# zgchen33/MCGaze

Hardware: AMD Instinct MI355X
Metric: clips/sec (7x3x224x224) (higher is better)
Workload: dtype f16x3; 1 GPU; full multiclue_gaze_r50 forward (R-50 + FPN + 4 decoder stages + gaze head), 64 clips/GPU x 7 frames x 3x224x224, 64 clips/step; clips_per_gpu=64, clip_length=7, global_clips=64, chunk_frames=0, parallelism=single GPU, trunk_streams=2

## Files before the change

include/mcgaze_hip.h:

```cpp
#ifndef MCGAZE_HIP_H
#define MCGAZE_HIP_H

#include <stddef.h>
#include <stdint.h>

#ifdef __cplusplus
extern "C" {
#endif

#define MCG_ABI_VERSION 19

enum { MCG_OK = 0, MCG_ERR_ARG = 1, MCG_ERR_HIP = 2, MCG_ERR_UNSUPPORTED = 3, MCG_ERR_WORKSPACE = 4 };
typedef enum { MCG_F32 = 0, MCG_BF16 = 1, MCG_F16X3 = 2, MCG_F16 = 3 } mcg_dtype;
#define MCG_ELEM_BYTES(dt) (((dt) == MCG_BF16 || (dt) == MCG_F16) ? 2 : 4)
typedef void* mcg_stream;

int mcg_abi_version(void);
const char* mcg_build_id(void);
const char* mcg_last_error(void);
int mcg_device_info(int* cu_count, size_t* hbm_bytes, char* arch, int arch_len);

int mcg_nchw_to_nhwc(mcg_stream s, mcg_dtype dt, const float* src, void* dst, int N, int C, int H, int W);
int mcg_nhwc_to_nchw(mcg_stream s, mcg_dtype dt, const void* src, float* dst, int N, int C, int H, int W);

// ... 11 lines not shown
  void* y;
  int N, H, W, Cin, Cout, KH, KW, stride, pad;
  int relu;
  int residual_mode;
  int Hr, Wr;
  const void* x2;
  int Cin2, stride2, H2, W2;
  int tile;
  int flags;
  float wscale;
} mcg_conv_desc;
int mcg_conv2d(mcg_stream s, mcg_dtype dt, const mcg_conv_desc* d);

int mcg_bottleneck_x3(mcg_stream s, const float* x, const float* src2, const void* wstream, const float* bias, float* y, float* z,
                      int frames, int H, int W, int cm, int nsrc, int cn, void* trace);

size_t mcg_conv3x3_wino_x3_weight_bytes(int Cin, int Cout, int g);
int mcg_conv3x3_wino_x3(mcg_stream s, const float* x, const void* u, const float* bias, float* y, int frames, int H, int W,
                        int Cin, int Cout, int relu, int tile, float wscale, int g);

int mcg_pointwise_stream(mcg_stream s, mcg_dtype dt, const void* a, const void* wf, const float* bias, const void* res, void* y,
                         int M, int K, int N, int relu, int res_mode, int Ho, int Wo, int Hr, int Wr, float wscale,
                         const int* block_list, const int* block_count, int grid_cap);
int mcg_pointwise_dyn(mcg_stream s, mcg_dtype dt, const void* a, const void* wf, const float* bias, void* y, int M, float wscale, int grid_cap);
int mcg_pointwise_pair(mcg_stream s, mcg_dtype dt, const void* a1, const void* a2, const void* res, const void* w3f, const float* b3,
                       void* y, const void* w1f, const float* b1, void* z, int M, int K2, int C2, int grid_cap);

size_t mcg_stem_workspace_bytes(mcg_dtype dt, int N, int H, int W);
int mcg_stem_forward(mcg_stream s, mcg_dtype dt, const float* img, const void* w_stem, const float* bias,
                     void* y, int N, int H, int W, void* ws, size_t ws_bytes, int flags);
// ... 268 lines not shown
```

mcgaze_amd/csrc/bneck_x3.hpp:

```cpp
#pragma once
#include "igemm_dma.hpp"

#ifndef BNX_ABLATE
#define BNX_ABLATE 0
#endif
namespace bnx {
constexpr int TH = 8, TW = 28, WH = TH + 2, WW = TW + 2;
constexpr int NPIX = TH * TW, NG = NPIX / 32, WPIX = WH * WW;
constexpr int PLANE = WPIX * 16 + 32;
constexpr int NPLANE = 16;
constexpr int WIN_BYTES = NPLANE * PLANE;
constexpr int SLAB = 16384, NSLOT = 5, RING_BYTES = NSLOT * SLAB;
constexpr int NCOMP = NG, NT = 64 * (NCOMP + 1);
constexpr int WIN_ROUNDS = (WPIX * 16 + NCOMP * 64 - 1) / (NCOMP * 64);
static_assert(NPIX % 32 == 0, "tile must be whole 32-pixel groups");
}

struct BneckParams {
  const float* x;
  const float* res;
  const char* wstream;
  const float* bias;
  float* y;
  float* z;
  int H, W, tiles_x, tiles_per_frame, total_tiles;
  int res_blocked, y_blocked;
  unsigned long long* trace;
};

__device__ __forceinline__ void bnx_split8(const float (&v)[8], bf16x8& hi, bf16x8& lo) {
  uint32_t h[4], l[4];
#pragma unroll
  for (int q = 0; q < 4; ++q) split_pair(v[2 * q], v[2 * q + 1], h[q], l[q]);
  hi = __builtin_bit_cast(bf16x8, make_uint4(h[0], h[1], h[2], h[3]));
  lo = __builtin_bit_cast(bf16x8, make_uint4(l[0], l[1], l[2], l[3]));
}

__device__ __forceinline__ void bnx_step(const char* sl, const bf16x8& xh, const bf16x8& xl, f32x16& a0, f32x16& a1) {
  const bf16x8 w0h = __builtin_bit_cast(bf16x8, *(const uint4*)(sl));
  const bf16x8 w0l = __builtin_bit_cast(bf16x8, *(const uint4*)(sl + 1024));
  const bf16x8 w1h = __builtin_bit_cast(bf16x8, *(const uint4*)(sl + 8192));
  const bf16x8 w1l = __builtin_bit_cast(bf16x8, *(const uint4*)(sl + 8192 + 1024));
// ... 1 lines not shown
  a1 = x3_mfma(w1l, xh, a1);
  a0 = x3_mfma(w0h, xl, a0);
  a1 = x3_mfma(w1h, xl, a1);
  a0 = x3_mfma(w0h, xh, a0);
  a1 = x3_mfma(w1h, xh, a1);
}

__device__ __forceinline__ void bnx_barrier_drained() {
  asm volatile("s_waitcnt lgkmcnt(0)" ::: "memory");
  __builtin_amdgcn_s_barrier();
}

template <int CM, int NSRC, int CN, int LAYOUT>
__global__ __launch_bounds__(bnx::NT, 1) void bneck_x3_kernel(const BneckParams p) {
  using namespace bnx;
  constexpr bool RES_BLK = (LAYOUT & 1) != 0, Y_BLK = (LAYOUT & 2) != 0;
  static_assert(!RES_BLK || NSRC == 1, "only a residual can arrive blocked");
  constexpr int C = 4 * CM, KH = CM / 64, NCH = C / 64;
  constexpr int PARTS = CM / 64 + NSRC - 1;
  constexpr int NS1 = 9 * KH * KH;
  constexpr int NS = NS1 + NCH * (PARTS + CN / 64);
  constexpr int CT1 = CM / 32, CT3 = CN / 32;
  constexpr int WPC = (WIN_ROUNDS + NCH - 1) / NCH;
  constexpr int RD = 1;
  static_assert(NCH % RD == 0, "chunk loop is unrolled by the prefetch depth");
  static_assert(CM == 64 || CM == 128, "64 or 128 mid channels");
  static_assert(NSRC == 1 || CM == 64, "the second source is layer1's first block only");
  extern __shared__ __attribute__((aligned(16))) char smem[];
  char* const s_win = smem;
  char* const s_ring = smem + WIN_BYTES;
  float* const s_bias = (float*)(smem + WIN_BYTES + RING_BYTES);
  const int tid = threadIdx.x, lane = tid & 63;
  const int wave = __builtin_amdgcn_readfirstlane(tid >> 6);
  for (int i = tid; i < CM + C + CN + 4; i += NT) s_bias[i] = p.bias[i];
  __syncthreads();
  const int first = blockIdx.x, stride = gridDim.x;
  if (first >= p.total_tiles) return;

  if (wave == NCOMP) {
    const u32x4 srd_w = make_srd(p.wstream);
    const uint32_t ring_base = (uint32_t)(uintptr_t)(__attribute__((address_space(3))) char*)s_ring;
    const uint32_t voff = (uint32_t)lane * 16u;
    uint32_t kt_issue = 0, slot_issue = 0;
    int issued_total = 0;
    auto issue = [&]() {
      const uint32_t src = kt_issue * SLAB, dst = ring_base + slot_issue * SLAB;
      if (!(BNX_ABLATE & 1) || issued_total < NSLOT || p.H < 0)
        static_for<16>([&](auto pc) { lds_dma16<decltype(pc)::value * 1024>(voff, srd_w, src + decltype(pc)::value * 1024, dst); });
      if (BNX_ABLATE & 1) ++issued_total;
// ... 53 lines not shown
    ty0 = tyi * TH;
    tx0 = (r - tyi * p.tiles_x) * TW;
  };
  auto win_load = [&](int t, int kh, int it) -> float4 {
    int n, ty0, tx0;
    origin(t, n, ty0, tx0);
    const int idx = it * (NCOMP * 64) + ctid;
    const int wp = idx >> 4, c16 = idx & 15;
    const int wy = wp / WW, wx = wp - wy * WW;
    const int gy = ty0 - 1 + wy, gx = tx0 - 1 + wx;
    float4 v = make_float4(0.f, 0.f, 0.f, 0.f);
    if (idx < WPIX * 16 && (unsigned)gy < (unsigned)p.H && (unsigned)gx < (unsigned)p.W)
      v = *(const float4*)(p.x + (((long long)n * p.H + gy) * p.W + gx) * CM + kh * 64 + c16 * 4);
    return v;
  };
  auto win_park = [&](int it, const float4& v) {
    const int idx = it * (NCOMP * 64) + ctid;
    if (idx >= WPIX * 16) return;
    const int wp = idx >> 4, c16 = idx & 15;
    uint32_t h0, l0, h1, l1;
    split_pair(v.x, v.y, h0, l0);
    split_pair(v.z, v.w, h1, l1);
    char* dst = s_win + (((c16 >> 2) * 2 + ((c16 >> 1) & 1)) * 2) * PLANE + wp * 16 + (c16 & 1) * 8;
    *(uint2*)dst = make_uint2(h0, h1);
    *(uint2*)(dst + PLANE) = make_uint2(l0, l1);
  };

  for (int it = 0; it < WIN_ROUNDS; ++it) win_park(it, win_load(first, 0, it));

  const uint32_t a_lane = (uint32_t)lane * 16u;
  uint32_t slot = 0;
  auto slab_at = [&](int i) { const uint32_t t = slot + i; return s_ring + (t >= NSLOT ? t - NSLOT : t) * SLAB + a_lane; };
  auto slab_adv = [&](int n) { slot = slot + n >= NSLOT ? slot + n - NSLOT : slot + n; };

  int tr_c = 0;
  auto stamp = [&]() {
    if (p.trace && blockIdx.x == 0 && tid == 0 && tr_c < 2040) { p.trace[tr_c] = __builtin_amdgcn_s_memtime(); ++tr_c; }
  };
  for (int tile = first; tile < p.total_tiles; tile += stride) {
    stamp();
    int n, ty0, tx0;
    origin(tile, n, ty0, tx0);
    const int gy = ty0 + ty, gx = tx0 + tx;
    const bool valid = gy < p.H && gx < p.W;
    const bool st_ok = valid && ((BNX_ABLATE & 4) ? p.H < 0 : true), ld_ok = valid && ((BNX_ABLATE & 2) ? p.H < 0 : true);
    const long long row = ((long long)n * p.H + (valid ? gy : 0)) * p.W + (valid ? gx : 0);
    const long long sblk = ((long long)tile * NG + g) * (32 * C);
    const uint32_t lane_off = (uint32_t)(pl * 8 + 4 * half);
    const int next = tile + stride;
    const bool has_next = next < p.total_tiles && ((BNX_ABLATE & 8) ? p.H < 0 : true);

    float4 rres[RD][2][4];
    bf16x8 xfh[4], xfl[4];
    auto res_load = [&](auto slotc, int chunk) {
      constexpr int SL = decltype(slotc)::value;
#pragma unroll
      for (int c = 0; c < 2; ++c)
#pragma unroll
        for (int q = 0; q < 4; ++q)
          rres[SL][c][q] = !ld_ok ? make_float4(0.f, 0.f, 0.f, 0.f)
                                  : (RES_BLK ? *(const float4*)(p.res + sblk + lane_off + chunk * 2048 + c * 1024 + q * 256)
                                                   : *(const float4*)(p.res + row * C + chunk * 64 + c * 32 + 8 * q + 4 * half));
    };
// ... 2 lines not shown
    } else {
#pragma unroll
      for (int s = 0; s < 4; ++s) {
        const float4 a = valid ? *(const float4*)(p.res + row * 64 + 16 * s + 4 * half) : make_float4(0.f, 0.f, 0.f, 0.f);
        const float4 b = valid ? *(const float4*)(p.res + row * 64 + 16 * s + 4 * half + 8) : make_float4(0.f, 0.f, 0.f, 0.f);
        const float v[8] = {a.x, a.y, a.z, a.w, b.x, b.y, b.z, b.w};
        bnx_split8(v, xfh[s], xfl[s]);
      }
    }

    float4 w2nd[KH == 2 ? WIN_ROUNDS : 1];
    const bool win2 = (BNX_ABLATE & 8) ? (p.H < 0 || tile == first) : true;
    if constexpr (KH == 2) {
      if (win2) {
#pragma unroll
        for (int it = 0; it < WIN_ROUNDS; ++it) w2nd[it] = win_load(tile, 1, it);
      }
    }
    f32x16 acc1[CT1];
#pragma unroll
    for (int c = 0; c < CT1; ++c)
#pragma unroll
      for (int r = 0; r < 16; ++r) acc1[c][r] = 0.f;
    asm volatile("s_waitcnt lgkmcnt(0)" ::: "memory");
    static_for<KH>([&](auto khc) {
      constexpr int KHI = decltype(khc)::value;
      if constexpr (KHI == 1) {
        bnx_barrier_drained();
        if (win2) {
#pragma unroll
          for (int it = 0; it < WIN_ROUNDS; ++it) win_park(it, w2nd[it]);
        }
        asm volatile("s_waitcnt lgkmcnt(0)" ::: "memory");
      }
      static_for<9>([&](auto tc) {
        constexpr int TAP = decltype(tc)::value;
        constexpr int TOFF = ((TAP / 3) * WW + TAP % 3) * 16;
        bnx_barrier_drained();
        const char* sl[CM / 64];
#pragma unroll
        for (int op = 0; op < CM / 64; ++op) sl[op] = slab_at(op);
        static_for<4>([&](auto jc) {
          constexpr int J = decltype(jc)::value;
          const bf16x8 xh = __builtin_bit_cast(bf16x8, *(const uint4*)(bw + (4 * J) * PLANE + TOFF));
          const bf16x8 xl = __builtin_bit_cast(bf16x8, *(const uint4*)(bw + (4 * J + 1) * PLANE + TOFF));
          static_for<CM / 64>([&](auto opc) {
            constexpr int OP = decltype(opc)::value;
            bnx_step(sl[OP] + J * 2048, xh, xl, acc1[2 * OP], acc1[2 * OP + 1]);
          });
        });
        slab_adv(CM / 64);
      });
    });
    stamp();
    bf16x8 tfh[CM / 16], tfl[CM / 16];
#pragma unroll
    for (int s = 0; s < CM / 16; ++s) {
      const int c = s >> 1, q0 = 2 * (s & 1);
      float v[8];
#pragma unroll
// ... 9 lines not shown

    f32x16 acc3[CT3 > 0 ? CT3 : 1];
#pragma unroll
    for (int c = 0; c < (CT3 > 0 ? CT3 : 1); ++c)
#pragma unroll
      for (int r = 0; r < 16; ++r) acc3[c][r] = 0.f;
#pragma unroll 1
    for (int oc0 = 0; oc0 < NCH; oc0 += RD)
    static_for<RD>([&](auto occ) {
      constexpr int SLOT = decltype(occ)::value;
      const int oc = oc0 + SLOT;
      float4 wv[WPC];
      if (has_next) {
#pragma unroll
        for (int j = 0; j < WPC; ++j)
          if (oc * WPC + j < WIN_ROUNDS) wv[j] = win_load(next, 0, oc * WPC + j);
      }
      f32x16 acc2[2];
#pragma unroll
      for (int c = 0; c < 2; ++c)
#pragma unroll
        for (int r = 0; r < 16; ++r) acc2[c][r] = 0.f;
      bnx_barrier_drained();
      static_for<PARTS>([&](auto pc) {
        constexpr int PART = decltype(pc)::value;
        const char* sl = slab_at(PART);
        static_for<4>([&](auto sc) {
          constexpr int S = decltype(sc)::value;
          const bf16x8 bh = PART < CM / 64 ? tfh[(PART < CM / 64 ? PART : 0) * 4 + S] : xfh[S];
          const bf16x8 bl = PART < CM / 64 ? tfl[(PART < CM / 64 ? PART : 0) * 4 + S] : xfl[S];
          bnx_step(sl + S * 2048, bh, bl, acc2[0], acc2[1]);
// ... 70 lines not shown
static inline int launch_bneck_x3_t(hipStream_t s, const BneckParams& p) {
  constexpr int kLds = bnx::WIN_BYTES + bnx::RING_BYTES + (CM + 4 * CM + CN + 4) * 4;
  int cus;
  if (kernel_ready<bneck_x3_kernel<CM, NSRC, CN, LAYOUT>>(kLds, &cus)) return 1;
  const int grid = p.total_tiles < cus ? p.total_tiles : cus;
  hipLaunchKernelGGL((bneck_x3_kernel<CM, NSRC, CN, LAYOUT>), dim3(grid), dim3(bnx::NT), kLds, s, p);
  return hipGetLastError() == hipSuccess ? 0 : 1;
}
static inline bool bneck_x3_layout_ok(int cm, int nsrc, int cn, int res_blocked, int y_blocked) {
  return (!res_blocked || nsrc == 1) && (!y_blocked || (cn == cm));
}
static inline int launch_bneck_x3(hipStream_t s, BneckParams p, int frames, int cm, int nsrc, int cn) {
  const int tiles_y = (p.H + bnx::TH - 1) / bnx::TH;
  p.tiles_x = (p.W + bnx::TW - 1) / bnx::TW;
  p.tiles_per_frame = tiles_y * p.tiles_x;
  const long long total = (long long)p.tiles_per_frame * frames;
  if (total <= 0 || total > 0x7fffffffLL) return 1;
  p.total_tiles = (int)total;
  if (!bneck_x3_layout_ok(cm, nsrc, cn, p.res_blocked, p.y_blocked)) return 1;
  const int lay = (p.res_blocked ? 1 : 0) | (p.y_blocked ? 2 : 0);
  if (cm == 128) {
    if (cn == 0) return lay ? launch_bneck_x3_t<128, 1, 0, 1>(s, p) : launch_bneck_x3_t<128, 1, 0, 0>(s, p);
    switch (lay) {
      case 0: return launch_bneck_x3_t<128, 1, 128, 0>(s, p);
      case 1: return launch_bneck_x3_t<128, 1, 128, 1>(s, p);
      case 2: return launch_bneck_x3_t<128, 1, 128, 2>(s, p);
      default: return launch_bneck_x3_t<128, 1, 128, 3>(s, p);
    }
  }
  if (nsrc == 1) {
    if (cn == 0) return lay ? launch_bneck_x3_t<64, 1, 0, 1>(s, p) : launch_bneck_x3_t<64, 1, 0, 0>(s, p);
    if (cn == 128) return lay ? launch_bneck_x3_t<64, 1, 128, 1>(s, p) : launch_bneck_x3_t<64, 1, 128, 0>(s, p);
    switch (lay) {
      case 0: return launch_bneck_x3_t<64, 1, 64, 0>(s, p);
      case 1: return launch_bneck_x3_t<64, 1, 64, 1>(s, p);
      case 2: return launch_bneck_x3_t<64, 1, 64, 2>(s, p);
      default: return launch_bneck_x3_t<64, 1, 64, 3>(s, p);
    }
  }
  if (cn == 0) return launch_bneck_x3_t<64, 2, 0, 0>(s, p);
  if (cn == 64) return lay ? launch_bneck_x3_t<64, 2, 64, 2>(s, p) : launch_bneck_x3_t<64, 2, 64, 0>(s, p);
  return launch_bneck_x3_t<64, 2, 128, 0>(s, p);
// ... 2 lines not shown
```

mcgaze_amd/csrc/engine.hip:

```cpp
#include "igemm.hpp"
#include "pw_pair.hpp"
#include "pw_single.hpp"
#include "bneck_x3.hpp"
#include "pw_single_x3.hpp"
#include "wino_x3.hpp"

#include <stdarg.h>
#include <stdlib.h>
#include <string.h>

#include <map>
#include <mutex>
#include <string>
#include <vector>

int launch_roi_align(hipStream_t s, mcg_dtype dt, const void* const feats[4], const int feat_h[4], const int feat_w[4],
                     const int strides[4], int C, const float* boxes, int num_boxes, int boxes_per_frame, const int32_t* frame_of,
                     int pyramid_frames, void* out, int32_t* levels_out);
int launch_init_queries(hipStream_t s, mcg_dtype dt, const float* init_boxes, const void* init_feats, const int* img_hw,
                        const int32_t* frame_of, int pyramid_frames, int H, int W, float* boxes, void* obj, int N);
bool roi_mark_supported(int H, int W);
int launch_defer_clear(hipStream_t s, int* p, int n);
int launch_roi_mark(hipStream_t s, const float* boxes, int num_boxes, int boxes_per_frame, int level, int H, int W, int stride, int* state,
                    int* list, int* count);
int launch_inner_mark(hipStream_t s, const int* out_list, const int* out_count, int H, int W, int nblk, int* state, int* list, int* count);

struct mcg_engine {
  mcg_dtype dt;
  int blocks[4];
  mcg_conv_weights stem;
  std::vector<mcg_conv_weights> convs;
  mcg_conv_weights lateral[4], fpn_out[4], c3_ds[4];
  std::vector<mcg_fused_block> fused;
  bool bneck_fused = true;
  bool bneck_blocked = true;
  int winograd = 1;
  int wino_tile = -1;
  int fpn_deferred = 1;
  int fpn_lateral_deferred = 1;
  static constexpr int kAuditCap = 256;
  unsigned long long* audit_dev = nullptr;
  std::vector<std::string> audit_names;
  const float* init_boxes;
  const void* init_feats;
  int num_stages;
  std::vector<const void*> stage_w;
  const void* gaze_w[MCG_GW_COUNT];
  float stds[4];
  static constexpr int kMaxSplit = 4, kCandidates = 8;
  struct StreamPool* pool = nullptr;
// ... 120 lines not shown
extern "C" int mcg_engine_set_option(mcg_engine* e, const char* name, int value) {
  MCG_CHECK_ARG(e && name, "mcg_engine_set_option: null pointer");
  std::lock_guard<std::mutex> lock(e->mu);
  if (!strcmp(name, "trunk_streams")) { MCG_CHECK_ARG(value >= 1 && value <= mcg_engine::kMaxSplit, "trunk_streams must be 1..%d", mcg_engine::kMaxSplit); e->trunk_streams = value; }
  else if (!strcmp(name, "max_range_frames")) { MCG_CHECK_ARG(value >= 0, "max_range_frames must be >= 0"); e->max_range_frames = value; }
  else if (!strcmp(name, "tile")) e->ctx.tile = value > 0 ? value : -1;
  else if (!strcmp(name, "staged_gemm")) e->ctx.staged = value != 0;
  else if (!strcmp(name, "conv3x3_c64")) e->ctx.c64 = value != 0;
  else if (!strcmp(name, "stem_fused")) e->ctx.stem_fused = value != 0;
  else if (!strcmp(name, "decoder_chain")) e->ctx.chain = value != 0;
  else if (!strcmp(name, "decoder_attn_block")) e->ctx.attn_block = value != 0;
  else if (!strcmp(name, "pointwise_pair")) e->pw_pair = value != 0;
  else if (!strcmp(name, "pointwise_stream")) e->pw_single = value != 0;
  else if (!strcmp(name, "bottleneck_fused")) e->bneck_fused = value != 0;
  else if (!strcmp(name, "bottleneck_blocked")) e->bneck_blocked = value != 0;
  else if (!strcmp(name, "winograd")) { MCG_CHECK_ARG(value >= 0 && value <= 2, "winograd must be 0, 1 or 2"); e->winograd = value; }
  else if (!strcmp(name, "fpn_deferred")) e->fpn_deferred = value != 0;
  else if (!strcmp(name, "fpn_lateral_deferred")) e->fpn_lateral_deferred = value != 0;
  else if (!strcmp(name, "wino_tile")) { MCG_CHECK_ARG(value >= -1 && value <= 3, "wino_tile must be -1 (by grid size) .. 3"); e->wino_tile = value; }
  else if (!strcmp(name, "range_audit")) {
    MCG_CHECK_ARG(!mcg_is16(e->dt) || !value, "range_audit: f32-storage engines only (MCG_F32, MCG_F16X3)");
    if (value && !e->audit_dev) {
      if (hipMalloc((void**)&e->audit_dev, sizeof(unsigned long long) * 2 * mcg_engine::kAuditCap) != hipSuccess) { e->audit_dev = nullptr; mcg_set_error("range_audit: hipMalloc failed"); return MCG_ERR_HIP; }
    }
    if (value && hipMemset(e->audit_dev, 0, sizeof(unsigned long long) * 2 * mcg_engine::kAuditCap) != hipSuccess) { mcg_set_error("range_audit: hipMemset failed"); return MCG_ERR_HIP; }
    if (!value && e->audit_dev) { (void)hipFree(e->audit_dev); e->audit_dev = nullptr; }
    e->audit_names.clear();
  }
  else { mcg_set_error("mcg_engine_set_option: unknown option '%s'", name); return MCG_ERR_ARG; }
  return MCG_OK;
// ... 195 lines not shown
  const bool ds = b == 0;
  const mcg_conv_weights &d2 = e->convs[ci + 1], &d3 = e->convs[ci + 2];
  const int kk = ds ? e->convs[ci + 3].cin : 0, ss = ds ? e->convs[ci + 3].stride : 1;
  const int cn_i = ci + (ds ? 4 : 3);
  const bool nx = f->cn == 0 || (cn_i < (int)e->convs.size() && e->convs[cn_i].k == 1 && e->convs[cn_i].stride == 1 && e->convs[cn_i].cout == f->cn && e->convs[cn_i].cin == f->c);
  return (d2.k == 3 && d2.stride == 1 && d2.pad == 1 && d2.cin == f->cm && d2.cout == f->cm && d3.cout == f->c && f->nsrc == (ds ? 2 : 1) && nx &&
          bneck_x3_applicable(f->cm, f->c, f->cn, f->nsrc, kk, ss)) ? f : nullptr;
}
static int fused_tail_step(const mcg_engine* e, hipStream_t s, const TrunkWs& t, AuditCursor& au, TrunkCursor& c, const mcg_fused_block* fb,
                           int n, int l, int b, void* y) {
  const bool has_ds = b == 0;
  const int k2 = has_ds ? e->convs[c.ci + 3].cin : 0;
  BneckParams bp;
  memset(&bp, 0, sizeof(bp));
  bp.x = (const float*)c.o1; bp.res = (const float*)c.x; bp.wstream = (const char*)fb->wstream; bp.bias = fb->bias;
  bp.y = (float*)y; bp.z = (float*)c.o2; bp.H = c.h; bp.W = c.w;
  const long long blk_bytes = (long long)n * ((c.h + bnx::TH - 1) / bnx::TH) * ((c.w + bnx::TW - 1) / bnx::TW) * bnx::NPIX * fb->c * (long long)esize(e->dt);
  const mcg_fused_block* fnext = (b + 1 < e->blocks[l]) ? fused_tail_at(e, c.ci + (has_ds ? 4 : 3), b + 1) : nullptr;
  bp.res_blocked = c.x_blocked ? 1 : 0;
  bp.y_blocked = (e->bneck_blocked && !e->audit_dev && y != (void*)t.c[l] && fb->cn > 0 && fnext && fnext->nsrc == 1 && fnext->c == fb->c &&
                  blk_bytes <= (long long)t.big) ? 1 : 0;
  const double M = (double)n * c.h * c.w;
  ProfRec* rec = prof_begin(e->ctx, s, 70, n * c.h * c.w, fb->c + fb->cn, 9 * fb->cm + fb->cm + k2 + fb->c,
                            2.0 * M * (9.0 * fb->cm * fb->cm + (double)(fb->cm + k2) * fb->c + (double)fb->c * fb->cn),
                            4.0 * (M * (fb->cm + (has_ds ? k2 : fb->c) + fb->c + fb->cn) + 9.0 * fb->cm * fb->cm + (double)(fb->cm + k2) * fb->c + (double)fb->c * fb->cn));
  MCG_TRY(launch_done(rec, s, launch_bneck_x3(s, bp, n, fb->cm, fb->nsrc, fb->cn), "bneck_x3"));
  audit_tensor(au, y, (long long)n * c.h * c.w * fb->c, "layer%d.%d.out (fused tail)", l + 1, b);
  if (fb->cn > 0) {
    audit_tensor(au, c.o2, (long long)n * c.h * c.w * fb->cn, "layer%d.%d.next_conv1 (fused tail)", l + 1, b);
    std::swap(c.o1, c.o2);
    c.o1_ready = true;
// ... 252 lines not shown
      if (hipStreamWaitEvent(si[i], e->ev_fork, 0) != hipSuccess) { mcg_set_error("mcg_backbone_fpn_forward: hipStreamWaitEvent failed"); return MCG_ERR_HIP; }
  }
  const size_t part_ws = k > 1 ? al256(trunk_layout(e->dt, per, H, W, nullptr).total) : 0;
  int rc = MCG_OK;
  for (int f0 = 0, i = 0; f0 < N && rc == MCG_OK; f0 += per, i = (i + 1) % k)
    rc = trunk_chunk(e, si[i], img, f0, (N - f0) < per ? (N - f0) : per, H, W, pyramid, (char*)ws + (size_t)i * part_ws, backbone_only, tk);
  for (int i = 1; i < k; ++i) {
    if (hipEventRecord(e->ev_join[i - 1], si[i]) != hipSuccess || hipStreamWaitEvent(s, e->ev_join[i - 1], 0) != hipSuccess) {
      mcg_set_error("mcg_backbone_fpn_forward: join failed");
      rc = rc == MCG_OK ? MCG_ERR_HIP : rc;
    }
  }
  return rc;
}

extern "C" int mcg_bottleneck_x3(mcg_stream s, const float* x, const float* src2, const void* wstream, const float* bias, float* y, float* z,
                                 int frames, int H, int W, int cm, int nsrc, int cn, void* trace) {
  MCG_CHECK_ARG(x && src2 && wstream && bias && y && (z || cn == 0), "mcg_bottleneck_x3: null pointer");
  MCG_CHECK_ARG(frames > 0 && H > 0 && W > 0, "mcg_bottleneck_x3: empty problem");
  MCG_CHECK_ARG(bneck_x3_applicable(cm, 4 * cm, cn, nsrc, 64, 1), "mcg_bottleneck_x3: unsupported shape (cm=%d nsrc=%d cn=%d)", cm, nsrc, cn);
  BneckParams bp;
  memset(&bp, 0, sizeof(bp));
  bp.x = x; bp.res = src2; bp.wstream = (const char*)wstream; bp.bias = bias; bp.y = y; bp.z = z; bp.H = H; bp.W = W; bp.trace = (unsigned long long*)trace;
  if (launch_bneck_x3((hipStream_t)s, bp, frames, cm, nsrc, cn)) { mcg_set_error("mcg_bottleneck_x3: launch failed"); return MCG_ERR_HIP; }
  return MCG_OK;
}

extern "C" size_t mcg_conv3x3_wino_x3_weight_bytes(int Cin, int Cout, int g) {
  return (Cin > 0 && Cout > 0 && Cin % 32 == 0 && Cout % wnx::UNT == 0 && (g == 2 || g == 4)) ? wino_x3_weight_bytes(Cin, Cout, g) : 0;
}
extern "C" int mcg_conv3x3_wino_x3(mcg_stream s, const float* x, const void* u, const float* bias, float* y, int frames, int H, int W,
                                   int Cin, int Cout, int relu, int tile, float wscale, int g) {
  MCG_CHECK_ARG(x && u && y, "mcg_conv3x3_wino_x3: null pointer");
  MCG_CHECK_ARG(tile >= 0 && tile <= 4, "mcg_conv3x3_wino_x3: tile must be 0 (by grid size) .. 4");
  if (!wino_x3_applicable(frames, H, W, Cin, Cout, g)) {
    mcg_set_error("mcg_conv3x3_wino_x3: unsupported shape (frames=%d %dx%d, %d -> %d channels, F(%d,3)): Cin %% 32, Cout %% 128, W <= 62 (F(4,3): W %% 4 == 0, W >= 16), a tile's window within its buffer", frames, H, W, Cin, Cout, g);
    return MCG_ERR_UNSUPPORTED;
  }
  WinoParams wp;
  memset(&wp, 0, sizeof(wp));
// ... 236 lines not shown
```

mcgaze_amd/engine.py:

```python
import ctypes as C
import os

import numpy as np
import torch

from . import lib as L
from .packing import PackedWeights

_TORCH_DT = {'bf16': torch.bfloat16, 'f16': torch.float16, 'fp16': torch.float16, 'fp32': torch.float32, 'f32': torch.float32, 'f16x3': torch.float32, 'bf16x3': torch.float32}
_CODE = {'bf16': L.MCG_BF16, 'f16': L.MCG_F16, 'fp16': L.MCG_F16, 'fp32': L.MCG_F32, 'f32': L.MCG_F32, 'f16x3': L.MCG_F16X3,
         'bf16x3': L.MCG_F16X3}


def _code(dtype):
    return L.MCG_BF16 if dtype == torch.bfloat16 else (L.MCG_F16 if dtype == torch.float16 else L.MCG_F32)


def _ptr(t):
    return C.c_void_p(t.data_ptr()) if t is not None else C.c_void_p(0)


def _stream(device=None):
    return C.c_void_p(torch.cuda.current_stream(device).cuda_stream)

# ... 107 lines not shown

def conv3x3_wino(x, w, bias=None, relu=False, tile=0, g=2):
    _require_gpu()
    lib = L.load()
    from .packing import pow2_prescale, wino_pack
    N, H, W, Cin = x.shape
    Cout = w.shape[0]
    ws, wscale = pow2_prescale(w.cpu())
    u = wino_pack(ws, g=g).to(x.device)
    assert u.numel() * 2 == lib.mcg_conv3x3_wino_x3_weight_bytes(Cin, Cout, g), (u.numel(), Cin, Cout)
    y = torch.empty(N, H, W, Cout, dtype=torch.float32, device=x.device)
    L.check(lib.mcg_conv3x3_wino_x3(_stream(), _ptr(x.contiguous()), _ptr(u), _ptr(bias), _ptr(y), N, H, W, Cin, Cout, int(relu), tile, wscale, g), 'mcg_conv3x3_wino_x3')
    return y


def bottleneck_x3(x, src2, wstream, bias, cn, nsrc, trace=None):
    _require_gpu()
    lib = L.load()
    N, H, W, cm = x.shape
    y = torch.empty(N, H, W, 4 * cm, dtype=torch.float32, device=x.device)
    z = torch.empty(N, H, W, cn, dtype=torch.float32, device=x.device) if cn else None
    L.check(lib.mcg_bottleneck_x3(_stream(), _ptr(x.contiguous()), _ptr(src2.contiguous()), _ptr(wstream), _ptr(bias), _ptr(y), _ptr(z),
                                  N, H, W, cm, nsrc, cn, _ptr(trace)), 'mcg_bottleneck_x3')
    return y, z


def stem(img, w_stem, bias, dtype, flags=0, split=False):
    _require_gpu()
    lib = L.load()
    N, _, H, W = img.shape
    code = L.MCG_F16X3 if split else _code(dtype)
    ws = _ws(lib.mcg_stem_workspace_bytes(code, N, H, W), img.device)
    y = torch.empty(N, H // 4, W // 4, 64, dtype=dtype, device=img.device)
    L.check(lib.mcg_stem_forward(_stream(), code, _ptr(img.contiguous()), _ptr(w_stem), _ptr(bias), _ptr(y), N, H, W,
                                 _ptr(ws), ws.numel(), flags), 'mcg_stem_forward')
    return y


# ... 454 lines not shown
```

mcgaze_amd/lib.py:

```python
import ctypes as C
import os

_HERE = os.path.dirname(os.path.abspath(__file__))
LIB_PATH = os.environ.get('MCGAZE_LIB') or os.path.join(_HERE, 'libmcgaze_hip.so')

MCG_OK = 0
MCG_F32, MCG_BF16, MCG_F16X3, MCG_F16 = 0, 1, 2, 3
ABI_VERSION = 19
RES_NONE, RES_ADD, RES_UPSAMPLE_ADD = 0, 1, 2
FLAG_STAGED_GEMM, FLAG_NO_SPECIALISED, FLAG_NO_ATTN_BLOCK = 1, 2, 4

STAGE_KEYS = [
    'IN_PROJ_W', 'IN_PROJ_B', 'OUT_PROJ_W', 'OUT_PROJ_B', 'ATTN_LN_G', 'ATTN_LN_B', 'DYN_W', 'DYN_B',
    'NORM_IN_G', 'NORM_IN_B', 'NORM_OUT_G', 'NORM_OUT_B', 'FC_W', 'FC_B', 'FC_LN_G', 'FC_LN_B', 'IIC_LN_G', 'IIC_LN_B',
    'FFN1_W', 'FFN1_B', 'FFN2_W', 'FFN2_B', 'FFN_LN_G', 'FFN_LN_B', 'CLS_FC_W', 'CLS_LN_G', 'CLS_LN_B',
    'REG_FC_W', 'REG_LN_G', 'REG_LN_B', 'HEAD_CLS_W', 'HEAD_CLS_B', 'HEAD_REG_W', 'HEAD_REG_B', 'OUT_PROJ_WF', 'CLS_FC_WF', 'REG_FC_WF', 'IN_PROJ_WF', 'DYN_WF']
GAZE_KEYS = ['FC_W', 'LN_G', 'LN_B', 'OUT_W', 'OUT_B', 'FUSE_W', 'FUSE_B']
SW_COUNT, GW_COUNT = len(STAGE_KEYS), len(GAZE_KEYS)

EXPORTS = ['mcg_abi_version', 'mcg_build_id', 'mcg_last_error', 'mcg_device_info', 'mcg_nchw_to_nhwc', 'mcg_nhwc_to_nchw', 'mcg_conv2d',
           'mcg_stem_workspace_bytes', 'mcg_stem_forward', 'mcg_roi_align', 'mcg_stage_workspace_bytes', 'mcg_stage_forward',
           'mcg_gaze_head_workspace_bytes', 'mcg_gaze_head', 'mcg_engine_create', 'mcg_engine_destroy',
           'mcg_engine_workspace_bytes', 'mcg_trunk_workspace_bytes', 'mcg_decoder_workspace_bytes', 'mcg_backbone_fpn_forward',
           'mcg_decoder_forward', 'mcg_clip_forward', 'mcg_preprocess_frames', 'mcg_engine_set_option', 'mcg_engine_profile_start',
           'mcg_engine_profile_stop', 'mcg_bench_backbone_forward', 'mcg_bottleneck_x3', 'mcg_bench_backbone_levels', 'mcg_conv3x3_wino_x3',
           'mcg_conv3x3_wino_x3_weight_bytes', 'mcg_engine_range_audit', 'mcg_roi_align_indexed', 'mcg_decoder_forward_indexed',
           'mcg_deferred_pyramid_bytes', 'mcg_deferred_pyramid_levels', 'mcg_backbone_fpn_forward_deferred', 'mcg_decoder_forward_deferred',
           'mcg_stage_forward_ragged', 'mcg_decoder_forward_ragged', 'mcg_decoder_forward_deferred_ragged', 'mcg_clip_forward_ragged',
           'mcg_pyramid_scatter_rows', 'mcg_preprocess_head_crops', 'mcg_merge_windows', 'mcg_smooth_gaze', 'mcg_preprocess_frames_nv12',
           'mcg_preprocess_head_crops_nv12', 'mcg_draw_gaze_arrows', 'mcg_draw_gaze_arrows_nv12',
           'mcg_detect_heads_workspace_bytes', 'mcg_detect_heads', 'mcg_letterbox_frames', 'mcg_letterbox_frames_nv12',
           'mcg_track_state_bytes', 'mcg_track_heads', 'mcg_track_heads_motion', 'mcg_live_slots', 'mcg_live_gate', 'mcg_live_lanes', 'mcg_live_gate_lanes',
           'mcg_deferred_pyramid_state', 'mcg_inner_block_neighbours', 'mcg_gaze_targets', 'mcg_gaze_dwell',
           'mcg_pointwise_stream', 'mcg_pointwise_dyn', 'mcg_pointwise_pair']
LETTERBOX_U8, LETTERBOX_F16, LETTERBOX_F32 = 0, 1, 2


class ConvDesc(C.Structure):
    _fields_ = [('x', C.c_void_p), ('w', C.c_void_p), ('bias', C.c_void_p), ('residual', C.c_void_p), ('y', C.c_void_p),
                ('N', C.c_int), ('H', C.c_int), ('W', C.c_int), ('Cin', C.c_int), ('Cout', C.c_int), ('KH', C.c_int),
                ('KW', C.c_int), ('stride', C.c_int), ('pad', C.c_int), ('relu', C.c_int), ('residual_mode', C.c_int),
                ('Hr', C.c_int), ('Wr', C.c_int), ('x2', C.c_void_p), ('Cin2', C.c_int), ('stride2', C.c_int), ('H2', C.c_int),
                ('W2', C.c_int), ('tile', C.c_int), ('flags', C.c_int), ('wscale', C.c_float)]


class ConvWeights(C.Structure):
    _fields_ = [('w', C.c_void_p), ('bias', C.c_void_p), ('cin', C.c_int), ('cout', C.c_int), ('k', C.c_int),
                ('stride', C.c_int), ('pad', C.c_int), ('wf', C.c_void_p), ('wscale', C.c_float), ('wf4', C.c_void_p)]

# ... 121 lines not shown
    lib.mcg_track_state_bytes.argtypes = [i, i]
    lib.mcg_track_heads.argtypes = [vp, vp, C.c_longlong, vp, i, i, i, i, C.c_double, i, vp, vp, vp, vp, vp, vp, vp]
    lib.mcg_track_heads_motion.argtypes = [vp, vp, C.c_longlong, vp, i, i, i, i, C.c_double, i, C.c_double, C.c_double, vp, vp, vp, vp, vp, vp, vp, vp]
    lib.mcg_live_slots.argtypes = [vp, vp, i, i, i, i, vp, vp, vp, vp, vp]
    lib.mcg_live_gate.argtypes = [vp, vp, vp, i, i, i, i, vp, i, i, i, vp, vp, vp, vp, vp, vp, vp, vp, vp]
    lib.mcg_live_lanes.argtypes = [vp, vp, i, i, i, i, i, vp, vp, vp, vp, vp, vp, vp, vp, vp]
    lib.mcg_live_gate_lanes.argtypes = [vp, vp, vp, vp, i, i, i, i, i, vp, i, i, i, vp, vp, vp, vp, vp, vp, vp, vp, vp, vp, vp]
    lib.mcg_gaze_targets.argtypes = [vp, vp, vp, i, vp, i, vp, vp, i, i, C.c_double, C.c_double, vp, vp, vp, vp, vp, vp]
    lib.mcg_gaze_dwell.argtypes = [vp, vp, vp, vp, vp, vp, i, i, i, i, i, vp, vp, i, vp, vp, vp, i, vp]
    lib.mcg_engine_set_option.argtypes = [vp, C.c_char_p, i]
    lib.mcg_engine_profile_start.argtypes = [vp, i]
    lib.mcg_engine_profile_stop.argtypes = [vp, C.POINTER(i), C.POINTER(C.c_float), C.POINTER(C.c_double), C.POINTER(C.c_double), C.POINTER(i), C.POINTER(i), i]
    lib.mcg_bench_backbone_forward.argtypes = [vp, vp, vp, i, i, i, vp, sz]
    lib.mcg_bench_backbone_levels.argtypes = [vp, vp, i, i, i, C.POINTER(vp)]
    lib.mcg_bottleneck_x3.argtypes = [vp, vp, vp, vp, vp, vp, vp, i, i, i, i, i, i, vp]
    lib.mcg_conv3x3_wino_x3.argtypes = [vp, vp, vp, vp, vp, i, i, i, i, i, i, i, C.c_float, i]
    lib.mcg_conv3x3_wino_x3_weight_bytes.restype = sz
    lib.mcg_pointwise_stream.argtypes = [vp, i, vp, vp, vp, vp, vp, i, i, i, i, i, i, i, i, i, C.c_float, vp, vp, i]
    lib.mcg_pointwise_dyn.argtypes = [vp, i, vp, vp, vp, vp, i, C.c_float, i]
    lib.mcg_pointwise_pair.argtypes = [vp, i, vp, vp, vp, vp, vp, vp, vp, vp, vp, i, i, i, i]
    lib.mcg_engine_range_audit.argtypes = [vp, C.POINTER(C.c_ulonglong), C.POINTER(C.c_char_p), i, C.POINTER(i)]
    lib.mcg_conv3x3_wino_x3_weight_bytes.argtypes = [i, i, i]
    for name in EXPORTS:
        fn = getattr(lib, name)
        if fn.restype is C.c_int and name not in ('mcg_abi_version',):
            fn.restype = i
    if lib.mcg_abi_version() != ABI_VERSION:
        raise McgError(f'ABI mismatch: library reports {lib.mcg_abi_version()}, binding expects {ABI_VERSION}')
    _lib = lib
    return lib
# ... 22 lines not shown
```

Baseline: 3620 clips/s.

## Pack half-empty last tile rows of frame pairs into shared layer2 bottleneck tiles

When the feature height leaves the last tile row half full (layer2 at 28x28), the fused bottleneck kernel now walks tiles so that the last half-rows of two consecutive frames share one tile. This removes the padded compute and weight streaming spent on empty rows, cutting the tile count per frame pair. It adds per-tile decode arithmetic, a zeroed LDS row for the halo seam between the two halves, and more template instantiations, at the risk of seam-handling bugs.

```diff
diff --git a/include/mcgaze_hip.h b/include/mcgaze_hip.h
--- a/include/mcgaze_hip.h
+++ b/include/mcgaze_hip.h
@@ -49,6 +49,8 @@
 
 int mcg_bottleneck_x3(mcg_stream s, const float* x, const float* src2, const void* wstream, const float* bias, float* y, float* z,
                       int frames, int H, int W, int cm, int nsrc, int cn, void* trace);
+int mcg_bottleneck_x3_layout(mcg_stream s, const float* x, const float* src2, const void* wstream, const float* bias, float* y, float* z,
+                             int frames, int H, int W, int cm, int nsrc, int cn, int flags, void* trace);
 
 size_t mcg_conv3x3_wino_x3_weight_bytes(int Cin, int Cout, int g);
 int mcg_conv3x3_wino_x3(mcg_stream s, const float* x, const void* u, const float* bias, float* y, int frames, int H, int W,
diff --git a/mcgaze_amd/csrc/bneck_x3.hpp b/mcgaze_amd/csrc/bneck_x3.hpp
--- a/mcgaze_amd/csrc/bneck_x3.hpp
+++ b/mcgaze_amd/csrc/bneck_x3.hpp
@@ -26,6 +26,12 @@
   int H, W, tiles_x, tiles_per_frame, total_tiles;
   int res_blocked, y_blocked;
   unsigned long long* trace;
+  int pair_rows;
+  int pairs, pair_wpp;
+};
+
+struct BnxOrg {
+  int n, ty0, tx0, tile, paired;
 };
 
 __device__ __forceinline__ void bnx_split8(const float (&v)[8], bf16x8& hi, bf16x8& lo) {
@@ -57,7 +63,8 @@
 template <int CM, int NSRC, int CN, int LAYOUT>
 __global__ __launch_bounds__(bnx::NT, 1) void bneck_x3_kernel(const BneckParams p) {
   using namespace bnx;
-  constexpr bool RES_BLK = (LAYOUT & 1) != 0, Y_BLK = (LAYOUT & 2) != 0;
+  constexpr bool RES_BLK = (LAYOUT & 1) != 0, Y_BLK = (LAYOUT & 2) != 0, PAIR = (LAYOUT & 4) != 0;
+  static_assert(!PAIR || CM == 128, "the paired tile walk is layer2's");
   static_assert(!RES_BLK || NSRC == 1, "only a residual can arrive blocked");
   constexpr int C = 4 * CM, KH = CM / 64, NCH = C / 64;
   constexpr int PARTS = CM / 64 + NSRC - 1;
@@ -76,6 +83,9 @@
   const int tid = threadIdx.x, lane = tid & 63;
   const int wave = __builtin_amdgcn_readfirstlane(tid >> 6);
   for (int i = tid; i < CM + C + CN + 4; i += NT) s_bias[i] = p.bias[i];
+  if constexpr (PAIR) {
+    if (tid < 2 * NPLANE) *(uint4*)(s_win + (tid >> 1) * PLANE + WPIX * 16 + (tid & 1) * 16) = make_uint4(0u, 0u, 0u, 0u);
+  }
   __syncthreads();
   const int first = blockIdx.x, stride = gridDim.x;
   if (first >= p.total_tiles) return;
@@ -159,6 +169,32 @@
       v = *(const float4*)(p.x + (((long long)n * p.H + gy) * p.W + gx) * CM + kh * 64 + c16 * 4);
     return v;
   };
+  auto decode = [&](int w) -> BnxOrg {
+    const int j = w / p.pair_wpp, r = w - j * p.pair_wpp, full = p.tiles_per_frame - p.tiles_x;
+    BnxOrg o;
+    o.paired = 0;
+    int rr = r;
+    if (j >= p.pairs) o.n = 2 * p.pairs;
+    else if (r < full) o.n = 2 * j;
+    else if (r < 2 * full) { o.n = 2 * j + 1; rr = r - full; }
+    else { o.n = 2 * j; rr = r - full; o.paired = 1; }
+    const int tyi = rr / p.tiles_x;
+    o.ty0 = tyi * TH;
+    o.tx0 = (rr - tyi * p.tiles_x) * TW;
+    o.tile = o.n * p.tiles_per_frame + rr;
+    return o;
+  };
+  auto win_load_o = [&](const BnxOrg& o, int kh, int it) -> float4 {
+    const int idx = it * (NCOMP * 64) + ctid;
+    const int wp = idx >> 4, c16 = idx & 15;
+    const int wy = wp / WW, wx = wp - wy * WW;
+    const bool second = o.paired && wy >= WH / 2;
+    const int gy = o.ty0 - 1 + (second ? wy - WH / 2 : wy), gx = o.tx0 - 1 + wx, n = o.n + (second ? 1 : 0);
+    float4 v = make_float4(0.f, 0.f, 0.f, 0.f);
+    if (idx < WPIX * 16 && (unsigned)gy < (unsigned)p.H && (unsigned)gx < (unsigned)p.W)
+      v = *(const float4*)(p.x + (((long long)n * p.H + gy) * p.W + gx) * CM + kh * 64 + c16 * 4);
+    return v;
+  };
   auto win_park = [&](int it, const float4& v) {
     const int idx = it * (NCOMP * 64) + ctid;
     if (idx >= WPIX * 16) return;
@@ -171,7 +207,12 @@
     *(uint2*)(dst + PLANE) = make_uint2(l0, l1);
   };
 
-  for (int it = 0; it < WIN_ROUNDS; ++it) win_park(it, win_load(first, 0, it));
+  if constexpr (PAIR) {
+    const BnxOrg o0 = decode(first);
+    for (int it = 0; it < WIN_ROUNDS; ++it) win_park(it, win_load_o(o0, 0, it));
+  } else {
+    for (int it = 0; it < WIN_ROUNDS; ++it) win_park(it, win_load(first, 0, it));
+  }
 
   const uint32_t a_lane = (uint32_t)lane * 16u;
   uint32_t slot = 0;
@@ -185,13 +226,28 @@
   for (int tile = first; tile < p.total_tiles; tile += stride) {
     stamp();
     int n, ty0, tx0;
-    origin(tile, n, ty0, tx0);
-    const int gy = ty0 + ty, gx = tx0 + tx;
+    BnxOrg org{}, org_next{};
+    bool second = false, last_row = false;
+    if constexpr (PAIR) {
+      org = decode(tile);
+      org_next = decode(tile + stride);
+      n = org.n; ty0 = org.ty0; tx0 = org.tx0;
+      second = org.paired && ty >= TH / 2;
+      last_row = org.paired && (ty & (TH / 2 - 1)) == TH / 2 - 1;
+      if (second) n += 1;
+    } else {
+      origin(tile, n, ty0, tx0);
+    }
+    const int gy = ty0 + ((PAIR && org.paired) ? (ty & (TH / 2 - 1)) : ty), gx = tx0 + tx;
     const bool valid = gy < p.H && gx < p.W;
+    const char* const bwt = (PAIR && second) ? bw + WW * 16 : bw;
+    const char* const bzero = s_win + half * 2 * PLANE + WPIX * 16;
     const bool st_ok = valid && ((BNX_ABLATE & 4) ? p.H < 0 : true), ld_ok = valid && ((BNX_ABLATE & 2) ? p.H < 0 : true);
     const long long row = ((long long)n * p.H + (valid ? gy : 0)) * p.W + (valid ? gx : 0);
-    const long long sblk = ((long long)tile * NG + g) * (32 * C);
-    const uint32_t lane_off = (uint32_t)(pl * 8 + 4 * half);
+    const int ml = (PAIR && second) ? m - NPIX / 2 : m;
+    const long long sblk = PAIR ? (long long)org.tile * NG * (32 * C) : ((long long)tile * NG + g) * (32 * C);
+    const uint32_t lane_off = PAIR ? (uint32_t)(((second ? p.tiles_per_frame * NG : 0) + (ml >> 5)) * (32 * C) + (ml & 31) * 8 + 4 * half)
+                                   : (uint32_t)(pl * 8 + 4 * half);
     const int next = tile + stride;
     const bool has_next = next < p.total_tiles && ((BNX_ABLATE & 8) ? p.H < 0 : true);
 
@@ -224,7 +280,10 @@
     if constexpr (KH == 2) {
       if (win2) {
 #pragma unroll
-        for (int it = 0; it < WIN_ROUNDS; ++it) w2nd[it] = win_load(tile, 1, it);
+        for (int it = 0; it < WIN_ROUNDS; ++it) {
+          if constexpr (PAIR) w2nd[it] = win_load_o(org, 1, it);
+          else w2nd[it] = win_load(tile, 1, it);
+        }
       }
     }
     f32x16 acc1[CT1];
@@ -250,10 +309,12 @@
         const char* sl[CM / 64];
 #pragma unroll
         for (int op = 0; op < CM / 64; ++op) sl[op] = slab_at(op);
+        const char* bt = bwt;
+        if constexpr (PAIR && TAP >= 6) bt = last_row ? bzero + (TAP == 6 ? 0 : 16) - TOFF : bwt;
         static_for<4>([&](auto jc) {
           constexpr int J = decltype(jc)::value;
-          const bf16x8 xh = __builtin_bit_cast(bf16x8, *(const uint4*)(bw + (4 * J) * PLANE + TOFF));
-          const bf16x8 xl = __builtin_bit_cast(bf16x8, *(const uint4*)(bw + (4 * J + 1) * PLANE + TOFF));
+          const bf16x8 xh = __builtin_bit_cast(bf16x8, *(const uint4*)(bt + (4 * J) * PLANE + TOFF));
+          const bf16x8 xl = __builtin_bit_cast(bf16x8, *(const uint4*)(bt + (4 * J + 1) * PLANE + TOFF));
           static_for<CM / 64>([&](auto opc) {
             constexpr int OP = decltype(opc)::value;
             bnx_step(sl[OP] + J * 2048, xh, xl, acc1[2 * OP], acc1[2 * OP + 1]);
@@ -293,7 +354,10 @@
       if (has_next) {
 #pragma unroll
         for (int j = 0; j < WPC; ++j)
-          if (oc * WPC + j < WIN_ROUNDS) wv[j] = win_load(next, 0, oc * WPC + j);
+          if (oc * WPC + j < WIN_ROUNDS) {
+            if constexpr (PAIR) wv[j] = win_load_o(org_next, 0, oc * WPC + j);
+            else wv[j] = win_load(next, 0, oc * WPC + j);
+          }
       }
       f32x16 acc2[2];
 #pragma unroll
@@ -394,18 +458,33 @@
   const int tiles_y = (p.H + bnx::TH - 1) / bnx::TH;
   p.tiles_x = (p.W + bnx::TW - 1) / bnx::TW;
   p.tiles_per_frame = tiles_y * p.tiles_x;
-  const long long total = (long long)p.tiles_per_frame * frames;
+  long long total = (long long)p.tiles_per_frame * frames;
   if (total <= 0 || total > 0x7fffffffLL) return 1;
+  const bool pair = p.pair_rows && cm == 128 && frames >= 2 && p.H % bnx::TH == bnx::TH / 2;
+  p.pairs = pair ? frames / 2 : 0;
+  p.pair_wpp = pair ? 2 * p.tiles_per_frame - p.tiles_x : 0;
+  if (pair) total = (long long)p.pairs * p.pair_wpp + (long long)(frames & 1) * p.tiles_per_frame;
   p.total_tiles = (int)total;
   if (!bneck_x3_layout_ok(cm, nsrc, cn, p.res_blocked, p.y_blocked)) return 1;
-  const int lay = (p.res_blocked ? 1 : 0) | (p.y_blocked ? 2 : 0);
+  const int lay = (p.res_blocked ? 1 : 0) | (p.y_blocked ? 2 : 0) | (pair ? 4 : 0);
   if (cm == 128) {
-    if (cn == 0) return lay ? launch_bneck_x3_t<128, 1, 0, 1>(s, p) : launch_bneck_x3_t<128, 1, 0, 0>(s, p);
+    if (cn == 0) {
+      switch (lay) {
+        case 0: return launch_bneck_x3_t<128, 1, 0, 0>(s, p);
+        case 1: return launch_bneck_x3_t<128, 1, 0, 1>(s, p);
+        case 4: return launch_bneck_x3_t<128, 1, 0, 4>(s, p);
+        default: return launch_bneck_x3_t<128, 1, 0, 5>(s, p);
+      }
+    }
     switch (lay) {
       case 0: return launch_bneck_x3_t<128, 1, 128, 0>(s, p);
       case 1: return launch_bneck_x3_t<128, 1, 128, 1>(s, p);
       case 2: return launch_bneck_x3_t<128, 1, 128, 2>(s, p);
-      default: return launch_bneck_x3_t<128, 1, 128, 3>(s, p);
+      case 3: return launch_bneck_x3_t<128, 1, 128, 3>(s, p);
+      case 4: return launch_bneck_x3_t<128, 1, 128, 4>(s, p);
+      case 5: return launch_bneck_x3_t<128, 1, 128, 5>(s, p);
+      case 6: return launch_bneck_x3_t<128, 1, 128, 6>(s, p);
+      default: return launch_bneck_x3_t<128, 1, 128, 7>(s, p);
     }
   }
   if (nsrc == 1) {
diff --git a/mcgaze_amd/csrc/engine.hip b/mcgaze_amd/csrc/engine.hip
--- a/mcgaze_amd/csrc/engine.hip
+++ b/mcgaze_amd/csrc/engine.hip
@@ -34,6 +34,7 @@
   std::vector<mcg_fused_block> fused;
   bool bneck_fused = true;
   bool bneck_blocked = true;
+  bool bneck_pair_rows = true;
   int winograd = 1;
   int wino_tile = -1;
   int fpn_deferred = 1;
@@ -184,6 +185,7 @@
   else if (!strcmp(name, "pointwise_stream")) e->pw_single = value != 0;
   else if (!strcmp(name, "bottleneck_fused")) e->bneck_fused = value != 0;
   else if (!strcmp(name, "bottleneck_blocked")) e->bneck_blocked = value != 0;
+  else if (!strcmp(name, "bneck_pair_rows")) e->bneck_pair_rows = value != 0;
   else if (!strcmp(name, "winograd")) { MCG_CHECK_ARG(value >= 0 && value <= 2, "winograd must be 0, 1 or 2"); e->winograd = value; }
   else if (!strcmp(name, "fpn_deferred")) e->fpn_deferred = value != 0;
   else if (!strcmp(name, "fpn_lateral_deferred")) e->fpn_lateral_deferred = value != 0;
@@ -409,7 +411,7 @@
   BneckParams bp;
   memset(&bp, 0, sizeof(bp));
   bp.x = (const float*)c.o1; bp.res = (const float*)c.x; bp.wstream = (const char*)fb->wstream; bp.bias = fb->bias;
-  bp.y = (float*)y; bp.z = (float*)c.o2; bp.H = c.h; bp.W = c.w;
+  bp.y = (float*)y; bp.z = (float*)c.o2; bp.H = c.h; bp.W = c.w; bp.pair_rows = e->bneck_pair_rows ? 1 : 0;
   const long long blk_bytes = (long long)n * ((c.h + bnx::TH - 1) / bnx::TH) * ((c.w + bnx::TW - 1) / bnx::TW) * bnx::NPIX * fb->c * (long long)esize(e->dt);
   const mcg_fused_block* fnext = (b + 1 < e->blocks[l]) ? fused_tail_at(e, c.ci + (has_ds ? 4 : 3), b + 1) : nullptr;
   bp.res_blocked = c.x_blocked ? 1 : 0;
@@ -692,16 +694,22 @@
   return rc;
 }
 
-extern "C" int mcg_bottleneck_x3(mcg_stream s, const float* x, const float* src2, const void* wstream, const float* bias, float* y, float* z,
-                                 int frames, int H, int W, int cm, int nsrc, int cn, void* trace) {
+extern "C" int mcg_bottleneck_x3_layout(mcg_stream s, const float* x, const float* src2, const void* wstream, const float* bias, float* y, float* z,
+                                        int frames, int H, int W, int cm, int nsrc, int cn, int flags, void* trace) {
   MCG_CHECK_ARG(x && src2 && wstream && bias && y && (z || cn == 0), "mcg_bottleneck_x3: null pointer");
   MCG_CHECK_ARG(frames > 0 && H > 0 && W > 0, "mcg_bottleneck_x3: empty problem");
   MCG_CHECK_ARG(bneck_x3_applicable(cm, 4 * cm, cn, nsrc, 64, 1), "mcg_bottleneck_x3: unsupported shape (cm=%d nsrc=%d cn=%d)", cm, nsrc, cn);
+  MCG_CHECK_ARG(!(flags & ~7) && bneck_x3_layout_ok(cm, nsrc, cn, flags & 1, flags & 2), "mcg_bottleneck_x3: flags %d do not fit the shape (cm=%d nsrc=%d cn=%d)", flags, cm, nsrc, cn);
   BneckParams bp;
   memset(&bp, 0, sizeof(bp));
   bp.x = x; bp.res = src2; bp.wstream = (const char*)wstream; bp.bias = bias; bp.y = y; bp.z = z; bp.H = H; bp.W = W; bp.trace = (unsigned long long*)trace;
+  bp.res_blocked = flags & 1; bp.y_blocked = (flags >> 1) & 1; bp.pair_rows = (flags & 4) ? 0 : 1;
   if (launch_bneck_x3((hipStream_t)s, bp, frames, cm, nsrc, cn)) { mcg_set_error("mcg_bottleneck_x3: launch failed"); return MCG_ERR_HIP; }
   return MCG_OK;
+}
+extern "C" int mcg_bottleneck_x3(mcg_stream s, const float* x, const float* src2, const void* wstream, const float* bias, float* y, float* z,
+                                 int frames, int H, int W, int cm, int nsrc, int cn, void* trace) {
+  return mcg_bottleneck_x3_layout(s, x, src2, wstream, bias, y, z, frames, H, W, cm, nsrc, cn, 0, trace);
 }
 
 extern "C" size_t mcg_conv3x3_wino_x3_weight_bytes(int Cin, int Cout, int g) {
diff --git a/mcgaze_amd/engine.py b/mcgaze_amd/engine.py
--- a/mcgaze_amd/engine.py
+++ b/mcgaze_amd/engine.py
@@ -145,14 +145,29 @@
     return y
 
 
-def bottleneck_x3(x, src2, wstream, bias, cn, nsrc, trace=None):
+BNECK_RES_BLOCKED, BNECK_Y_BLOCKED, BNECK_NO_PAIR_ROWS = 1, 2, 4
+
+
+def bneck_blocked_floats(N, H, W, c):
+    return N * ((H + 7) // 8) * ((W + 27) // 28) * 224 * c
+
+
+def bottleneck_x3(x, src2, wstream, bias, cn, nsrc, trace=None, flags=0, out=None):
     _require_gpu()
     lib = L.load()
     N, H, W, cm = x.shape
-    y = torch.empty(N, H, W, 4 * cm, dtype=torch.float32, device=x.device)
-    z = torch.empty(N, H, W, cn, dtype=torch.float32, device=x.device) if cn else None
-    L.check(lib.mcg_bottleneck_x3(_stream(), _ptr(x.contiguous()), _ptr(src2.contiguous()), _ptr(wstream), _ptr(bias), _ptr(y), _ptr(z),
-                                  N, H, W, cm, nsrc, cn, _ptr(trace)), 'mcg_bottleneck_x3')
+    if out is not None:
+        y, z = out
+        assert y.is_contiguous() and (z is None or z.is_contiguous())
+        assert y.numel() == (bneck_blocked_floats(N, H, W, 4 * cm) if flags & BNECK_Y_BLOCKED else N * H * W * 4 * cm)
+        assert (z is None) == (cn == 0) and (z is None or z.numel() == N * H * W * cn)
+    else:
+        y = (torch.empty(bneck_blocked_floats(N, H, W, 4 * cm), dtype=torch.float32, device=x.device) if flags & BNECK_Y_BLOCKED
+             else torch.empty(N, H, W, 4 * cm, dtype=torch.float32, device=x.device))
+        z = torch.empty(N, H, W, cn, dtype=torch.float32, device=x.device) if cn else None
+    assert src2.numel() == (bneck_blocked_floats(N, H, W, 4 * cm) if flags & BNECK_RES_BLOCKED else N * H * W * (4 * cm if nsrc == 1 else 64))
+    L.check(lib.mcg_bottleneck_x3_layout(_stream(), _ptr(x.contiguous()), _ptr(src2.contiguous()), _ptr(wstream), _ptr(bias), _ptr(y), _ptr(z),
+                                         N, H, W, cm, nsrc, cn, flags, _ptr(trace)), 'mcg_bottleneck_x3')
     return y, z
 
 
diff --git a/mcgaze_amd/lib.py b/mcgaze_amd/lib.py
--- a/mcgaze_amd/lib.py
+++ b/mcgaze_amd/lib.py
@@ -32,7 +32,7 @@
            'mcg_detect_heads_workspace_bytes', 'mcg_detect_heads', 'mcg_letterbox_frames', 'mcg_letterbox_frames_nv12',
            'mcg_track_state_bytes', 'mcg_track_heads', 'mcg_track_heads_motion', 'mcg_live_slots', 'mcg_live_gate', 'mcg_live_lanes', 'mcg_live_gate_lanes',
            'mcg_deferred_pyramid_state', 'mcg_inner_block_neighbours', 'mcg_gaze_targets', 'mcg_gaze_dwell',
-           'mcg_pointwise_stream', 'mcg_pointwise_dyn', 'mcg_pointwise_pair']
+           'mcg_pointwise_stream', 'mcg_pointwise_dyn', 'mcg_pointwise_pair', 'mcg_bottleneck_x3_layout']
 LETTERBOX_U8, LETTERBOX_F16, LETTERBOX_F32 = 0, 1, 2
 
 
@@ -184,6 +184,7 @@
     lib.mcg_bench_backbone_forward.argtypes = [vp, vp, vp, i, i, i, vp, sz]
     lib.mcg_bench_backbone_levels.argtypes = [vp, vp, i, i, i, C.POINTER(vp)]
     lib.mcg_bottleneck_x3.argtypes = [vp, vp, vp, vp, vp, vp, vp, i, i, i, i, i, i, vp]
+    lib.mcg_bottleneck_x3_layout.argtypes = [vp, vp, vp, vp, vp, vp, vp, i, i, i, i, i, i, i, vp]
     lib.mcg_conv3x3_wino_x3.argtypes = [vp, vp, vp, vp, vp, i, i, i, i, i, i, i, C.c_float, i]
     lib.mcg_conv3x3_wino_x3_weight_bytes.restype = sz
     lib.mcg_pointwise_stream.argtypes = [vp, i, vp, vp, vp, vp, vp, i, i, i, i, i, i, i, i, i, C.c_float, vp, vp, i]
```

Result: no change. 3643 clips/s (median of 6 runs) (+0.6%).
